# AndrewGYork/rescan_line_sted

Hardware: AMD Instinct MI355X
Metric: simulated frames/s (512x512, 20 RL iters) (higher is better)
Workload: dtype f32; 1 GPU; astronaut 128->512x512 (np.kron x4), point-descan STED PSF 107x107 (2.0x operating point), simulate (H + Philox Poisson) + 20 RL iterations per frame; n_psf=1, rl_iters=20, fft=576x576

## Files before the change

include/rlsted.h:

```cpp
#ifndef RLSTED_H
#define RLSTED_H

#include <stddef.h>
#include <stdint.h>

#ifdef __cplusplus
extern "C" {
#endif

#define RL_OK 0
#define RL_ERR_INVALID -1
#define RL_ERR_HIP -2
#define RL_ERR_UNSUPPORTED -3
#define RL_ERR_STATE -4

#define RL_F32 0
#define RL_F64 1

#define RL_RNG_NONE 0
#define RL_RNG_PHILOX 1

typedef struct rl_ctx rl_ctx;
typedef struct rl_deconv rl_deconv;
typedef struct rl_comm rl_comm;
// ... 44 lines not shown

int rl_deconv_get_object(rl_deconv* h, double* out);
int rl_deconv_get_noiseless(rl_deconv* h, double* out);
int rl_deconv_get_measurement(rl_deconv* h, double* out);
int rl_deconv_get_estimate(rl_deconv* h, double* out);
int rl_deconv_get_normalization(rl_deconv* h, double* out);

int rl_forward(rl_deconv* h, const double* x, double* out);
int rl_adjoint(rl_deconv* h, const double* y, double* out, int normalize);

int rl_deconv_last_ms(const rl_deconv* h, double* iterate_ms, double* simulate_ms);

int rl_deconv_bench_cycles(rl_deconv* h, int k, int reps, int rng_kind, uint64_t seed, double* total_ms);

int rl_deconv_device_ptr(rl_deconv* h, int which, void** ptr, size_t* n_elements, int* dtype);

int rl_deconv_measurement_written(rl_deconv* h);

int rl_deconv_strategy(const rl_deconv* h, int* separable, int* real_psf_spectrum, int* split_column_pass, int* frame_pairs);

int rl_deconv_object_classes(const rl_deconv* h, int* classes, int* shared_slices, int* slices);

int rl_deconv_simulated_images(const rl_deconv* h, int* images);

int rl_deconv_unresolved(rl_deconv* h, unsigned long long* count, int reset);

int rl_deconv_dims(const rl_deconv* h, int* batch, int* n_psf, int* ny, int* nx);

typedef struct rl_task {
    const double* object;
    double total_brightness;
    uint64_t seed;
    uint32_t image_id;
} rl_task;
int rl_batch_run(rl_deconv* h, const rl_task* tasks, int n_tasks, int k_iters, int rng_kind, double* estimates_out);

int rl_batch_submit(rl_deconv* h, const rl_task* tasks, int n_tasks, int k_iters, int rng_kind, void* dev_out, int out_dtype);

#define RL_TRACE_FIELDS 6
int rl_batch_submit_checkpoints(rl_deconv* h, const rl_task* tasks, int n_tasks, const int* k_list, int n_k, int rng_kind,
                                void* const* dev_out, int out_dtype, double* const* trace_dev);

int rl_device_alloc(rl_ctx* ctx, size_t bytes, void** dev_out);
int rl_device_free(rl_ctx* ctx, void* dev);
int rl_device_download(rl_ctx* ctx, const void* dev, int dtype, size_t n_elements, double* host_out);
int rl_device_upload(rl_ctx* ctx, void* dev, int dtype, size_t n_elements, const double* host);
// ... 121 lines not shown
```

rescan_line_sted_amd/_lib.py:

```python
import ctypes
import os

import numpy as np

_HERE = os.path.dirname(os.path.abspath(__file__))
LIB_PATH = os.environ.get('RLSTED_LIB') or os.path.join(_HERE, '_lib', 'librlsted.so')
DEFAULT_DEVICE = int(os.environ.get('RLSTED_DEVICE', '0'))

RL_F32, RL_F64 = 0, 1
RNG_NONE, RNG_PHILOX = 0, 1
DTYPES = {'f32': RL_F32, 'float32': RL_F32, 'f64': RL_F64, 'float64': RL_F64}
RL_ACCEL_NONE, RL_ACCEL_BIGGS_ANDREWS = 0, 1
ACCELERATIONS = {None: RL_ACCEL_NONE, 'none': RL_ACCEL_NONE, 'biggs-andrews': RL_ACCEL_BIGGS_ANDREWS}
RL_STOP_DISCREPANCY, RL_STOP_RELATIVE = 1, 2
STOP_RULES = {'discrepancy': RL_STOP_DISCREPANCY, 'relative': RL_STOP_RELATIVE}


def accel_mode(acceleration):
    try:
        return ACCELERATIONS[acceleration]
    except (KeyError, TypeError):
        raise ValueError("acceleration must be None or 'biggs-andrews'; got %r" % (acceleration,)) from None


# ... 32 lines not shown
    'rl_deconv_set_acceleration': (_i, [_vp, _i]),
    'rl_deconv_get_alpha': (_i, [_vp, _dp]),
    'rl_deconv_set_tv': (_i, [_vp, _c.c_double, _c.c_double]),
    'rl_deconv_get_tv': (_i, [_vp, _dp, _dp]),
    'rl_deconv_divergence': (_i, [_vp, _dp]),
    'rl_deconv_iterate_until': (_i, [_vp, _i, _i, _i, _c.c_double, _c.POINTER(_i), _dp, _c.POINTER(_i)]),
    'rl_deconv_get_object': (_i, [_vp, _dp]),
    'rl_deconv_get_noiseless': (_i, [_vp, _dp]),
    'rl_deconv_get_measurement': (_i, [_vp, _dp]),
    'rl_deconv_get_estimate': (_i, [_vp, _dp]),
    'rl_deconv_get_normalization': (_i, [_vp, _dp]),
    'rl_forward': (_i, [_vp, _dp, _dp]),
    'rl_adjoint': (_i, [_vp, _dp, _dp, _i]),
    'rl_deconv_last_ms': (_i, [_vp, _dp, _dp]),
    'rl_deconv_bench_cycles': (_i, [_vp, _i, _i, _i, _c.c_uint64, _dp]),
    'rl_deconv_time_kernels': (_i, [_vp, _i, _dp]),
    'rl_deconv_time_cycle': (_i, [_vp, _i, _i, _c.c_uint64, _dp, _dp, _dp]),
    'rl_deconv_device_ptr': (_i, [_vp, _i, _c.POINTER(_vp), _c.POINTER(_c.c_size_t), _c.POINTER(_i)]),
    'rl_host_alloc': (_i, [_c.c_size_t, _c.POINTER(_vp)]),
    'rl_host_free': (_i, [_vp]),
    'rl_deconv_strategy': (_i, [_vp, _c.POINTER(_i), _c.POINTER(_i), _c.POINTER(_i), _c.POINTER(_i)]),
    'rl_deconv_object_classes': (_i, [_vp, _c.POINTER(_i), _c.POINTER(_i), _c.POINTER(_i)]),
    'rl_deconv_simulated_images': (_i, [_vp, _c.POINTER(_i)]),
    'rl_deconv_unresolved': (_i, [_vp, _c.POINTER(_c.c_uint64), _i]),
    'rl_deconv_dims': (_i, [_vp, _c.POINTER(_i), _c.POINTER(_i), _c.POINTER(_i), _c.POINTER(_i)]),
    'rl_batch_run': (_i, [_vp, _vp, _i, _i, _i, _dp]),
    'rl_batch_submit': (_i, [_vp, _vp, _i, _i, _i, _vp, _i]),
    'rl_batch_submit_checkpoints': (_i, [_vp, _vp, _i, _c.POINTER(_i), _i, _i, _c.POINTER(_vp), _i, _c.POINTER(_vp)]),
    'rl_device_alloc': (_i, [_vp, _c.c_size_t, _c.POINTER(_vp)]),
    'rl_device_free': (_i, [_vp, _vp]),
    'rl_device_download': (_i, [_vp, _vp, _i, _c.c_size_t, _dp]),
    'rl_device_upload': (_i, [_vp, _vp, _i, _c.c_size_t, _dp]),
    'rl_comm_gather_device': (_i, [_vp, _vp, _c.POINTER(_c.c_size_t), _i, _i, _vp]),
    'rl_comm_bcast_host': (_i, [_vp, _dp, _c.c_size_t, _i]),
    'rl_comm_unique_id': (_i, [_vp]),
    'rl_comm_create': (_i, [_vp, _i, _i, _vp, _c.POINTER(_vp)]),
    'rl_comm_destroy': (_i, [_vp]),
    'rl_comm_info': (_i, [_vp, _c.POINTER(_i), _c.POINTER(_i)]),
    'rl_comm_barrier': (_i, [_vp]),
    'rl_comm_allreduce_max': (_i, [_vp, _dp]),
    'rl_gather': (_i, [_vp, _vp, _i, _i, _c.POINTER(_i), _dp]),
    'rl_gather_device': (_i, [_vp, _vp, _i, _i, _c.POINTER(_i), _c.POINTER(_vp), _c.POINTER(_c.c_size_t), _c.POINTER(_i)]),
    'rl_comm_gather_host': (_i, [_vp, _dp, _c.POINTER(_c.c_size_t), _i, _dp]),
    'rl_rotate_image': (_i, [_vp, _dp, _dp, _i, _i, _c.c_double, _i]),
    'rl_fig3_scan': (_i, [_vp, _vp, _dp, _dp, _c.POINTER(_i), _i, _c.POINTER(_i), _i, _dp, _dp, _dp, _dp]),
    'rl_gauss_fit': (_i, [_dp, _i, _dp, _c.POINTER(_i)]),
# ... 153 lines not shown

    def info(self):
        ly, lx, pitch, nbytes = _i(), _i(), _i(), _c.c_size_t()
        check(lib.rl_deconv_info(self.handle, ctypes.byref(ly), ctypes.byref(lx), ctypes.byref(pitch),
                                 ctypes.byref(nbytes)))
        return {'ly': ly.value, 'lx': lx.value, 'pitch': pitch.value, 'device_bytes': nbytes.value}

    def strategy(self):
        a, b, c, d = _i(), _i(), _i(), _i()
        check(lib.rl_deconv_strategy(self.handle, ctypes.byref(a), ctypes.byref(b), ctypes.byref(c), ctypes.byref(d)))
        return {'separable': a.value == 1, 'direct_stencil': a.value == 2, 'real_psf_spectrum': bool(b.value),
                'split_column_pass': bool(c.value), 'frame_pairs': bool(d.value)}

    def object_classes(self):
        a, b, c = _i(), _i(), _i()
        check(lib.rl_deconv_object_classes(self.handle, ctypes.byref(a), ctypes.byref(b), ctypes.byref(c)))
        return {'classes': a.value, 'shared_slices': b.value, 'slices': c.value}

    def simulated_images(self):
        a = _i()
        check(lib.rl_deconv_simulated_images(self.handle, ctypes.byref(a)))
        return a.value

    def set_object(self, obj, total_brightness=None):
        obj = as_f64(obj).reshape(self.B, self.ny, self.nx)
        tb = None
        if total_brightness is not None:
            tb = as_f64(np.broadcast_to(np.asarray(total_brightness, dtype=np.float64), (self.B,)))
        check(lib.rl_deconv_set_object(self.handle, ptr(obj), ptr(tb) if tb is not None else None))

    def simulate(self, seed=0, rng=RNG_PHILOX):
        check(lib.rl_deconv_simulate(self.handle, rng, _c.c_uint64(seed)))

    def unresolved(self, reset=False):
        n = _c.c_uint64(0)
        check(lib.rl_deconv_unresolved(self.handle, _c.byref(n), 1 if reset else 0))
        return int(n.value)

    def set_measurement(self, noisy):
        noisy = as_f64(noisy).reshape(self.B, self.V, self.ny, self.nx)
        check(lib.rl_deconv_set_measurement(self.handle, ptr(noisy)))

    def measurement_written(self):
        check(lib.rl_deconv_measurement_written(self.handle))

    def iterate(self, k=1):
# ... 175 lines not shown
```

rescan_line_sted_amd/csrc/aux_kernels.hip:

```cpp
#include <hip/hip_runtime.h>
#include "aux_kernels.hpp"
#include "philox_poisson.hpp"

namespace rl {

template <typename T>
__global__ void k_fill(T* p, size_t n, T value) {
    for (size_t i = (size_t)blockIdx.x * blockDim.x + threadIdx.x; i < n; i += (size_t)gridDim.x * blockDim.x) p[i] = value;
}

__global__ void k_psf_dft_rows(const double* __restrict__ psf, const double2* __restrict__ wx, double2* __restrict__ s1,
                               int py, int px, int lx, int kx) {
    const int k = blockIdx.x * blockDim.x + threadIdx.x;
    const int a = blockIdx.y, v = blockIdx.z;
    if (k >= kx) return;
    const int cx = (px - 1) / 2;
    const double* row = psf + ((size_t)v * py + a) * px;
    double re = 0.0, im = 0.0;
    for (int b = 0; b < px; ++b) {
        const int off = ((b - cx) % lx + lx) % lx;
        const double2 w = wx[(int)(((long long)k * off) % lx)];
        re += row[b] * w.x;
        im += row[b] * w.y;
    }
// ... 20 lines not shown
    if (transposed) {
        if (k < kx) out[((size_t)v * kx + k) * ly + ky] = mk<T>((T)(re * scale), (T)(im * scale));
    } else {
        out[((size_t)v * ly + ky) * pitch + k] = mk<T>((T)(re * scale), (T)(im * scale));
    }
}

struct PoissonKeys {
    unsigned long long seed0;
    unsigned image0, V;
    const unsigned long long* frame_seeds;
    const unsigned* frame_ids;
    const unsigned* rate_frame;
    __device__ __forceinline__ unsigned long long seed(unsigned img) const { return frame_seeds ? frame_seeds[img / V] : seed0; }
    __device__ __forceinline__ unsigned image(unsigned img) const {
        return frame_seeds ? frame_ids[img / V] * V + img % V : image0 + img;
    }
    template <typename T>
    __device__ __forceinline__ T rate(const T* __restrict__ noiseless, unsigned i, unsigned n_pix) const {
        if (!rate_frame) return noiseless[i];
        const unsigned img = i / n_pix, pix = i - img * n_pix;
        return noiseless[((size_t)rate_frame[img / V] * V + img % V) * n_pix + pix];
    }
};

constexpr int kPoissonE = 8, kPoissonTile = 256 * kPoissonE;
template <typename T>
__global__ void __launch_bounds__(256) k_poisson(const T* __restrict__ noiseless, T* __restrict__ noisy, unsigned n_pix, unsigned total,
                                                 PoissonKeys keys, int rng_kind) {
    __shared__ unsigned lst_idx[2][kPoissonTile];
    __shared__ T lst_lam[2][kPoissonTile];
    __shared__ unsigned cnt[2], cnt_small;
    const unsigned tid = threadIdx.x;
    for (unsigned tile0 = blockIdx.x * (unsigned)kPoissonTile; tile0 < total; tile0 += gridDim.x * (unsigned)kPoissonTile) {
        if (tid == 0) cnt[0] = cnt_small = 0;
        __syncthreads();
#pragma unroll
        for (int e = 0; e < kPoissonE; ++e) {
            const unsigned i = tile0 + tid + 256u * (unsigned)e;
            if (i < total) {
                const T lam_t = keys.rate(noiseless, i, n_pix);
                const double lam = (double)lam_t;
                if (rng_kind != 1) {
                    noisy[i] = (T)(lam + 1e-9);
                } else {
                    const unsigned img = i / n_pix, pix = i - img * n_pix;
                    double k;
                    if (philox_poisson_fast(lam, keys.seed(img), keys.image(img), pix, &k)) {
                        noisy[i] = (T)(k + 1e-9);
                    } else if (lam >= 10.0) {
                        const unsigned q = atomicAdd(&cnt[0], 1u);
                        lst_idx[0][q] = i;
                        lst_lam[0][q] = lam_t;
                    } else {
                        const unsigned q = kPoissonTile - 1u - atomicAdd(&cnt_small, 1u);
                        lst_idx[0][q] = i;
                        lst_lam[0][q] = lam_t;
                    }
                }
            }
        }
        __syncthreads();
        if (rng_kind != 1) continue;
        unsigned n = cnt[0];
        const unsigned n_small = cnt_small;
        int cur = 0;
        for (unsigned blk = 0; n > 0; ++blk) {
            if (tid == 0) cnt[cur ^ 1] = 0;
            __syncthreads();
            const bool last = blk + 1 == kPoissonMaxBlocks;
            for (unsigned q = tid; q < n; q += 256u) {
                const unsigned i = lst_idx[cur][q];
                const T lam_t = lst_lam[cur][q];
                const unsigned img = i / n_pix, pix = i - img * n_pix;
                const unsigned long long seed = keys.seed(img);
                double k;
                const bool done = philox_ptrs_attempt((double)lam_t, (unsigned)seed, (unsigned)(seed >> 32), keys.image(img), pix, blk, &k);
                if (done || last) {
                    noisy[i] = (T)((done || k >= 0.0 ? k : 0.0) + 1e-9);
                } else {
                    const unsigned q2 = atomicAdd(&cnt[cur ^ 1], 1u);
                    lst_idx[cur ^ 1][q2] = i;
                    lst_lam[cur ^ 1][q2] = lam_t;
                }
            }
            __syncthreads();
            n = cnt[cur ^ 1];
            cur ^= 1;
        }
        for (unsigned q = tid; q < n_small; q += 256u) {
            const unsigned at = kPoissonTile - 1u - q, i = lst_idx[0][at];
            const unsigned img = i / n_pix;
            noisy[i] = (T)(philox_poisson((double)lst_lam[0][at], keys.seed(img), keys.image(img), i - img * n_pix) + 1e-9);
        }
        __syncthreads();
    }
}

template <typename T>
__global__ void __launch_bounds__(1024) k_frame_sums(const T* __restrict__ x, size_t n, double* __restrict__ out) {
    __shared__ double part[16];
    const size_t chunks = gridDim.y, len = (n + chunks - 1) / chunks, i0 = blockIdx.y * len, i1 = i0 + len < n ? i0 + len : n;
    const T* f = x + (size_t)blockIdx.x * n;
    double v = 0.0;
    for (size_t i = i0 + threadIdx.x; i < i1; i += blockDim.x) v += (double)f[i];
    for (int off = 32; off > 0; off >>= 1) v += __shfl_down(v, off, 64);
    if ((threadIdx.x & 63) == 0) part[threadIdx.x >> 6] = v;
    __syncthreads();
    if (threadIdx.x < 64) {
        v = threadIdx.x < (blockDim.x >> 6) ? part[threadIdx.x] : 0.0;
        for (int off = 8; off > 0; off >>= 1) v += __shfl_down(v, off, 64);
        if (threadIdx.x == 0) out[(size_t)blockIdx.x * chunks + blockIdx.y] = v;
    }
}
template <typename T>
// ... 71 lines not shown
    if (e != hipSuccess) return e;
    const unsigned g = blocks_for(n, 256);
    if (dtype == DT_F32) k_split_real<float><<<g, 256, 0, s>>>((const cx<float>*)z, n, (float*)re, stats);
    else k_split_real<double><<<g, 256, 0, s>>>((const cx<double>*)z, n, (double*)re, stats);
    return hipGetLastError();
}

template <typename T>
__global__ void k_box_norm(const double* __restrict__ integ, T* __restrict__ out, int V, int py, int px, int ny, int nx) {
    const int j = blockIdx.x * blockDim.x + threadIdx.x, i = blockIdx.y;
    if (j >= nx) return;
    out[(size_t)i * nx + j] = box_norm_pixel<T>(integ, V, py, px, ny, nx, i, j);
}

hipError_t aux_box_norm(int dtype, const double* integral_dev, void* out, int V, int py, int px, int ny, int nx, hipStream_t s) {
    const dim3 grid((unsigned)((nx + 255) / 256), (unsigned)ny);
    if (dtype == DT_F32) k_box_norm<float><<<grid, 256, 0, s>>>(integral_dev, (float*)out, V, py, px, ny, nx);
    else k_box_norm<double><<<grid, 256, 0, s>>>(integral_dev, (double*)out, V, py, px, ny, nx);
    return hipGetLastError();
}

hipError_t aux_poisson(int dtype, const void* noiseless, void* noisy, unsigned n_pix, unsigned n_img, unsigned image0,
                       unsigned long long seed, int rng_kind, void* list_ws, hipStream_t s,
                       const unsigned long long* frame_seeds, const unsigned* frame_ids, unsigned V, const unsigned* rate_frame) {
    (void)list_ws;
    const PoissonKeys keys{seed, image0, V ? V : 1u, frame_seeds, frame_ids, rate_frame};
    const size_t total = (size_t)n_pix * n_img;
    if (total >= 0xffffffffull - (size_t)kPoissonTile * 4096) return hipErrorInvalidValue;
    if (total == 0) return hipSuccess;
    const size_t tiles = (total + kPoissonTile - 1) / kPoissonTile;
    const unsigned g = (unsigned)(tiles > 4096 ? 4096 : tiles);
    if (dtype == DT_F32) k_poisson<float><<<g, 256, 0, s>>>((const float*)noiseless, (float*)noisy, n_pix, (unsigned)total, keys, rng_kind);
    else k_poisson<double><<<g, 256, 0, s>>>((const double*)noiseless, (double*)noisy, n_pix, (unsigned)total, keys, rng_kind);
    return hipGetLastError();
}

hipError_t aux_scale_convert(int dtype, const double* src, void* dst, size_t n, size_t frames, const double* target,
                             double* sums, hipStream_t s, bool want_sums) {
    if (target || want_sums) frame_sums<double>(src, n, frames, sums, s);
    const unsigned g = blocks_for(n * frames, 256);
    if (dtype == DT_F32) k_scale_convert<float><<<g, 256, 0, s>>>(src, (float*)dst, n, frames, target, sums);
    else k_scale_convert<double><<<g, 256, 0, s>>>(src, (double*)dst, n, frames, target, sums);
    return hipGetLastError();
}

template <typename T>
__global__ void k_any_negative(const T* __restrict__ x, size_t n, int* __restrict__ flag) {
    bool neg = false;
    for (size_t i = (size_t)blockIdx.x * blockDim.x + threadIdx.x; i < n; i += (size_t)gridDim.x * blockDim.x) neg = neg || x[i] < (T)0;
    if (__any(neg) && (threadIdx.x & 63) == 0) atomicOr(flag, 1);
}
hipError_t aux_any_negative(int dtype, const void* src, size_t n, int* flag, hipStream_t s) {
    hipError_t e = hipMemsetAsync(flag, 0, sizeof(int), s);
    if (e != hipSuccess || n == 0) return e;
    const unsigned g = blocks_for(n, 256);
    if (dtype == DT_F32) k_any_negative<float><<<g, 256, 0, s>>>((const float*)src, n, flag);
// ... 74 lines not shown
```

rescan_line_sted_amd/csrc/aux_kernels.hpp:

```cpp
#pragma once
#include "fft_core.hpp"

#include <cstddef>

#if defined(__HIPCC__) || defined(__HIP_PLATFORM_AMD__)
#include <hip/hip_runtime.h>
#include "kernel_table.hpp"
#endif

namespace rl {

template <typename T>
RL_HD T box_norm_pixel(const double* __restrict__ integ, int V, int py, int px, int ny, int nx, int i, int j) {
    const int cy = (py - 1) / 2, cx = (px - 1) / 2;
    const int a0 = i + cy - ny + 1 > 0 ? i + cy - ny + 1 : 0, a1 = (i + cy < py - 1 ? i + cy : py - 1) + 1;
    const int b0 = j + cx - nx + 1 > 0 ? j + cx - nx + 1 : 0, b1 = (j + cx < px - 1 ? j + cx : px - 1) + 1;
    double acc = 0.0;
    if (a1 > a0 && b1 > b0) {
        for (int v = 0; v < V; ++v) {
            const double* I = integ + (size_t)v * (py + 1) * (px + 1);
            const double s = (I[(size_t)a1 * (px + 1) + b1] - I[(size_t)a0 * (px + 1) + b1]) - (I[(size_t)a1 * (px + 1) + b0] - I[(size_t)a0 * (px + 1) + b0]);
            acc += s > 0.0 ? s : 0.0;
        }
    }
    return (T)acc;
}

#if defined(__HIPCC__) || defined(__HIP_PLATFORM_AMD__)
hipError_t aux_fill(int dtype, void* p, size_t n, double value, hipStream_t s);
hipError_t aux_psf_spectrum(int dtype, const double* psf_dev, const void* wx_dev, const void* wy_dev, void* s1_dev,
                            void* out, int n_psf, int py, int px, int ly, int lx, int kx, int pitch, int transposed,
                            hipStream_t s);
size_t aux_poisson_workspace_bytes(size_t total_pixels);
hipError_t aux_poisson(int dtype, const void* noiseless, void* noisy, unsigned n_pix, unsigned n_img, unsigned image0,
                       unsigned long long seed, int rng_kind, void* list_ws, hipStream_t s,
                       const unsigned long long* frame_seeds = nullptr, const unsigned* frame_ids = nullptr, unsigned V = 1,
                       const unsigned* rate_frame = nullptr);
constexpr size_t kSumChunks = 64;
inline size_t aux_sums_elems(size_t frames) { return frames * (1 + kSumChunks); }
hipError_t aux_scale_convert(int dtype, const double* src, void* dst, size_t n, size_t frames, const double* target,
                             double* sums, hipStream_t s, bool want_sums = false);
hipError_t aux_any_negative(int dtype, const void* src, size_t n, int* flag, hipStream_t s);
hipError_t aux_image_sums(int dtype, const void* src, size_t n, size_t frames, double* sums, hipStream_t s);
hipError_t aux_scale_convert_indexed(int dtype, const double* src, const unsigned* idx, size_t n_unique, void* dst, size_t n, size_t frames,
                                     const double* target, double* sums, hipStream_t s);
hipError_t aux_to_f64(int dtype, const void* src, double* dst, size_t total, hipStream_t s);
hipError_t aux_cast(int dtype_src, const void* src, int dtype_dst, void* dst, size_t total, hipStream_t s);
hipError_t aux_gather_images(int dtype, const void* src, void* dst, const unsigned* list, size_t n, size_t images, unsigned V, hipStream_t s);
hipError_t aux_split_real(int dtype, const void* z, size_t n, void* re, double* stats, hipStream_t s);
hipError_t aux_box_norm(int dtype, const double* integral_dev, void* out, int V, int py, int px, int ny, int nx, hipStream_t s);
#endif
}
```

rescan_line_sted_amd/csrc/rlsted.cpp:

```cpp
#include "../../include/rlsted.h"

#include <hip/hip_runtime.h>

#include <cmath>
#include <cstdio>
#include <cstdlib>
#include <algorithm>
#include <cstring>
#include <map>
#include <string>
#include <vector>

#include "accel_kernels.hpp"
#include "aux_kernels.hpp"
#include "checkpoint_kernels.hpp"
#include "conv_kernels.hpp"
#include "kernel_table.hpp"
#include "object_classes.hpp"
#include "ctx.hpp"
#include "sep_kernels.hpp"
#include "sep_taps.hpp"
#include "stop_kernels.hpp"
#include "tv_kernels.hpp"

// ... 22 lines not shown

const KernelTable* table_for(int L) {
    switch (L) {
        case 64: return table_64();
        case 192: return table_192();
        case 256: return table_256();
        case 576: return table_576();
        case 1152: return table_1152();
        case 2304: return table_2304();
        case 4608: return table_4608();
    }
    return nullptr;
}
const int kLengths[] = {64, 192, 256, 576, 1152, 2304, 4608};

size_t esize(int dtype) { return dtype == RL_F32 ? 4 : 8; }

constexpr int kMaxLanes = 4;

struct PlanOptions {
    bool chunk_mb_set = false;
    double chunk_mb = 0;
    int lanes = 2;
    bool inplace = true;
    int col_order = 4;
    bool pair = false;
    double pair_max_ratio = 4.0;
    bool sub_one = false;
    int fuse_views = -1;
    bool col_split = true;
    bool real_psf = true;
    bool ones_shortcut = true;
    bool share_objects = true;
    int sep = 1;
    int sep_one = 1;
    int direct = 1;
    bool q_exp_est_set = false, q_exp_ratio_set = false;
    int q_exp_est = 14, q_exp_ratio = 14;
};

PlanOptions plan_options(int dtype, int n_psf) {
    PlanOptions o;
    auto flag = [](const char* name, bool unset) {
        const char* s = getenv(name);
        return s ? atoi(s) != 0 : unset;
    };
    auto number = [](const char* name, int unset, bool* set = nullptr) {
        const char* s = getenv(name);
        if (set) *set = s != nullptr;
        return s ? atoi(s) : unset;
    };
    if (const char* s = getenv("RLSTED_CHUNK_MB")) {
        o.chunk_mb_set = true;
        o.chunk_mb = atof(s);
    }
    o.lanes = std::min(std::max(number("RLSTED_LANES", o.lanes), 1), kMaxLanes);
    o.inplace = flag("RLSTED_INPLACE", o.inplace);
    o.col_order = std::max(number("RLSTED_COL_ORDER", o.col_order), 1);
    o.pair = flag("RLSTED_PAIR", dtype == RL_F32 && n_psf == 1);
    if (const char* s = getenv("RLSTED_PAIR_MAX_RATIO")) o.pair_max_ratio = atof(s);
    o.sub_one = flag("RLSTED_SUB_ONE", dtype == RL_F32 && RL_SPEC_QUANT == 0);
    if (const char* s = getenv("RLSTED_FUSE_VIEWS")) o.fuse_views = atoi(s) != 0 ? 1 : 0;
    o.col_split = flag("RLSTED_COL_SPLIT", o.col_split);
    o.real_psf = flag("RLSTED_REAL_PSF", o.real_psf);
    o.ones_shortcut = flag("RLSTED_ONES_SHORTCUT", o.ones_shortcut);
    o.share_objects = flag("RLSTED_SHARE_OBJECTS", o.share_objects);
    o.sep = number("RLSTED_SEP", o.sep);
    o.sep_one = number("RLSTED_SEP_ONE", o.sep_one);
    o.direct = number("RLSTED_DIRECT", o.direct);
    o.q_exp_est = number("RLSTED_Q_EXP_EST", o.q_exp_est, &o.q_exp_est_set);
    o.q_exp_ratio = number("RLSTED_Q_EXP_RATIO", o.q_exp_ratio, &o.q_exp_ratio_set);
    return o;
}

struct TempBuffers {
    std::vector<void*> bufs;
    int get(void** p, size_t bytes) {
        HIP_TRY(hipMalloc(p, bytes));
        bufs.push_back(*p);
// ... 588 lines not shown
        if (c > 8) {
            const int up = (c + 7) / 8 * 8;
            c = up <= fit ? up : std::max(8, fit / 8 * 8);
        }
        if (pair && (c & 1)) ++c;
        return c >= B ? B : c;
    }
    int start_estimate_chunk(int f0, int nf, bool with_spectrum = true) {
        HIP_TRY(aux_fill(dtype, off(est, (size_t)f0 * n_img()), (size_t)nf * n_img(), 1.0, cur()));
        if (with_spectrum && pair)
            RL_TRY(row_pair(ROW_FWD, nf, nullptr, pair_spec(f0), off(est, (size_t)f0 * n_img()), nullptr, nullptr));
        else if (with_spectrum && !sep)
            RL_TRY(row(ROW_FWD, (unsigned)nf, nullptr, off(spec_a, (size_t)f0 * n_spec() * 2), off(est, (size_t)f0 * n_img()),
                       nullptr, nullptr));
        return RL_OK;
    }
    int ensure_lanes() {
        if (fork) return RL_OK;
        HIP_TRY(hipEventCreateWithFlags(&fork, hipEventDisableTiming));
        for (int l = 0; l < opt.lanes; ++l) {
            HIP_TRY(hipStreamCreateWithFlags(&lane_stream[l], hipStreamNonBlocking));
            HIP_TRY(hipEventCreateWithFlags(&lane_done[l], hipEventDisableTiming));
            HIP_TRY(hipEventCreateWithFlags(&lane_drawn[l], hipEventDisableTiming));
        }
        HIP_TRY(hipEventCreateWithFlags(&rates_ready, hipEventDisableTiming));
        return RL_OK;
    }
    bool one_buffer() const { return V == 1 && opt.inplace; }
    void* est_spec(int f0) const { return pair ? pair_spec(f0) : off(spec_a, (size_t)f0 * n_spec() * 2); }
    void* ratio_spec(int f0) const { return pair || one_buffer() ? est_spec(f0) : off(spec_b, (size_t)f0 * V * n_spec() * 2); }
    void* parked(int f0) const { return off(spec_x, (size_t)f0 * V * n_spec_x() * 2); }
    bool ht_fused() const { return fuse_views && V > 1 && (col_split() || wave_private_y()); }
    int pass_h(const Iter& it) {
        if (it.first) return RL_OK;
        if (pair) return col_pair(est_spec(it.f0), ratio_spec(it.f0), (it.nf + 1) / 2, COL_H, &it);
        if (col_split() && split_h()) return col_split_pass(est_spec(it.f0), ratio_spec(it.f0), parked(it.f0), it.nf, COL_H, &it);
        return col(est_spec(it.f0), ratio_spec(it.f0), it.nf, COL_H, &it);
    }
    int pass_ratio(const Iter& it) {
        void* r = ratio_spec(it.f0);
        const void* m = off(meas, (size_t)it.f0 * V * n_img());
        if (pair) return row_pair(ROW_RATIO, it.nf, it.first ? spec_ones_pair : r, r, m, nullptr, nullptr, it.first ? 1 : 0, 1, &it);
        return row(ROW_RATIO, (unsigned)(it.nf * V), it.first ? spec_ones : r, r, m, nullptr, nullptr, nullptr, -1, it.first ? V : 0, &it);
    }
    int pass_ht(const Iter& it) {
        void* r = ratio_spec(it.f0);
// ... 30 lines not shown
        if (col_split()) RL_TRY(col_split_pass(sa, sb, parked(f0), nf, COL_H));
        else RL_TRY(col(sa, sb, nf, COL_H));
        RL_TRY(row(ROW_INV, (unsigned)(nf * V), sb, nullptr, nullptr, out, nullptr));
        return RL_OK;
    }
    std::vector<int> obj_class;
    int n_classes = 0;
    std::vector<SliceShare> share_slices;
    int share_cf = 0;
    std::vector<uint32_t> share_reps, share_rate;
    struct ShareLists { const unsigned *rep_frames, *rate_of; };
    ShareLists share_lists{nullptr, nullptr};
    unsigned* share_dev = nullptr;
    void *obj_c = nullptr, *noiseless_c = nullptr;
    void *cls_spec_a = nullptr, *cls_spec_b = nullptr, *cls_spec_x = nullptr;
    size_t share_cap = 0;
    int share_classes = 0;
    hipEvent_t rates_ready = nullptr;
    hipEvent_t lane_drawn[kMaxLanes] = {nullptr, nullptr, nullptr, nullptr};
    bool lane_drawn_set[kMaxLanes] = {false, false, false, false};
    int last_sim_images = 0;
    bool noiseless_sparse = false;
    int last_shared_slices = 0, last_slices = 0;
    bool share_possible() const { return opt.share_objects && !sep && (int)obj_class.size() == B && n_classes < B; }
    int build_share(int cf, const ShareLists* staged) {
        share_cf = 0;
        noiseless_sparse = false;
        share_classes = 0;
        share_layout(obj_class, cf, share_slices, share_reps, share_rate);
        const size_t total = (size_t)class_layout(obj_class, cf, share_slices, share_reps, share_rate);
        if (total > share_cap) {
            HIP_TRY(hipDeviceSynchronize());
            share_cap = 0;
            RL_TRY(release(&obj_c));
            RL_TRY(release(&noiseless_c));
            RL_TRY(release(&cls_spec_a));
            RL_TRY(release(&cls_spec_b));
            RL_TRY(release(&cls_spec_x));
            const size_t cap = (total + 7) / 8 * 8, sp = n_spec() * 2 * esize(dtype);
            RL_TRY(alloc(&obj_c, cap * n_img() * esize(dtype), SLACK));
            RL_TRY(alloc(&noiseless_c, cap * V * n_img() * esize(dtype), SLACK));
            if (!pair_layout) RL_TRY(alloc(&cls_spec_a, cap * sp, SLACK));
            RL_TRY(alloc(&cls_spec_b, cap * V * sp, SLACK));
            if (col_split()) {
                const size_t parked_bytes = cap * V * n_spec_x() * 2 * esize(dtype);
                RL_TRY(alloc(&cls_spec_x, parked_bytes));
// ... 66 lines not shown
        const int frames = std::min(f0 + nf, cp.nt) - f0;
        void* dst = cp.out ? cp.out[j] : nullptr;
        double* tr = cp.trace ? cp.trace[j] : nullptr;
        if (frames <= 0 || (!dst && !tr)) return RL_OK;
        const size_t o = (size_t)f0 * n_img();
        double* part = tr ? cp_part + (size_t)f0 * checkpoint_blocks(n_img(), esize(dtype)) * kCheckpointFields : nullptr;
        HIP_TRY(checkpoint_take(dtype, off(est, o), off(obj, o), cp.out_dtype, dst ? (char*)dst + o * esize(cp.out_dtype) : nullptr, part,
                                n_img(), frames, cur()));
        if (tr) HIP_TRY(checkpoint_totals(dtype, part, n_img(), frames, tr + (size_t)f0 * kCheckpointFields, cur()));
        return RL_OK;
    }
    int run_slices(int k, bool restart, const Draw* draw = nullptr, bool cycle_follows = false, const Checkpoints* cp = nullptr) {
        const int cf = chunk_frames();
        const int slices = (B + cf - 1) / cf;
        const int nl = slices < opt.lanes ? slices : opt.lanes;
        const bool keep_open = cycle_follows && nl > 1;
        if (accel && restart) RL_TRY(accel_reset());
        if (draw && share_possible() && share_cf != cf && !lanes_open) RL_TRY(build_share(cf, nullptr));
        const bool share = draw && share_possible() && share_cf == cf;
        if (nl > 1 && !lanes_open) {
            RL_TRY(ensure_lanes());
            HIP_TRY(hipEventRecord(fork, ctx->stream));
            for (int l = 0; l < nl; ++l) HIP_TRY(hipStreamWaitEvent(lane_stream[l], fork, 0));
        }
        if (draw) {
            const size_t stride = (aux_poisson_workspace_bytes((size_t)cf * V * n_img()) + 255) / 256 * 256;
            if (slice_ws_bytes < stride * slices) {
                HIP_TRY(hipDeviceSynchronize());
                slice_ws_bytes = 0;
                RL_TRY(release(&slice_ws));
                RL_TRY(alloc(&slice_ws, stride * slices));
                slice_ws_bytes = stride * slices;
            }
            slice_ws_stride = stride;
        }
        int rc = RL_OK;
        struct ActiveGuard {
            hipStream_t& a;
            ~ActiveGuard() { a = nullptr; }
        } active_guard{active};
        int shared_slices = 0, sim_images = 0;
        auto hip_rc = [&](hipError_t e, const char* what) -> int {
            return e == hipSuccess ? RL_OK : fail(RL_ERR_HIP, std::string(what) + ": " + hipGetErrorString(e));
        };
        bool lane_waits[kMaxLanes] = {false, false, false, false};
        int lane_last_shared[kMaxLanes] = {-1, -1, -1, -1};
        if (share && share_classes > 0) {
            active = nl > 1 ? lane_stream[0] : nullptr;
            for (int l = 0; l < kMaxLanes && rc == RL_OK; ++l) {
                if (!lane_drawn_set[l]) continue;
                lane_drawn_set[l] = false;
                rc = hip_rc(hipStreamWaitEvent(cur(), lane_drawn[l], 0), "class simulation");
            }
            if (rc == RL_OK) rc = forward_classes(share_classes);
            sim_images += share_classes * V;
            if (nl > 1 && rc == RL_OK) {
                rc = hip_rc(hipEventRecord(rates_ready, cur()), "class simulation");
                for (int l = 1; l < nl; ++l) lane_waits[l] = true;
                for (int sl = 0; sl < slices; ++sl)
                    if (share_slices[(size_t)sl].nrep > 0) lane_last_shared[sl % nl] = sl;
            }
        }
        auto simulate_slice = [&](int sl, int f0, int nf) -> int {
            const SliceShare ss = share ? share_slices[(size_t)sl] : SliceShare{};
            const void* rates = off(noiseless, (size_t)f0 * V * n_img());
            const int lane = nl > 1 ? sl % nl : 0;
            if (ss.nrep > 0) {
                if (lane_waits[lane]) {
                    HIP_TRY(hipStreamWaitEvent(cur(), rates_ready, 0));
                    lane_waits[lane] = false;
                }
                rates = noiseless_c;
                ++shared_slices;
            } else {
                RL_TRY(forward_slice(f0, nf));
                sim_images += nf * V;
            }
            void* ws = (char*)slice_ws + (size_t)sl * slice_ws_stride;
            TimedScope t(this, TK_POISSON, false);
            hipError_t e = aux_poisson(dtype, rates, off(meas, (size_t)f0 * V * n_img()),
                                       (unsigned)n_img(), (unsigned)(nf * V), (unsigned)(f0 * V), draw->seed, draw->rng_kind, ws, cur(),
                                       draw->key_seeds ? draw->key_seeds + f0 : nullptr, draw->key_ids ? draw->key_ids + f0 : nullptr, (unsigned)V,
                                       ss.nrep > 0 ? share_lists.rate_of + f0 : nullptr);
            if (e != hipSuccess) return fail(RL_ERR_HIP, std::string("Poisson kernels: ") + hipGetErrorString(e));
            if (lane_last_shared[lane] == sl) {
                HIP_TRY(hipEventRecord(lane_drawn[lane], cur()));
                lane_drawn_set[lane] = true;
            }
            return RL_OK;
        };
        for (int sl = 0, f0 = 0; f0 < B && rc == RL_OK; f0 += cf, ++sl) {
            const int nf = f0 + cf <= B ? cf : B - f0;
            active = nl > 1 ? lane_stream[sl % nl] : nullptr;
            if (draw) rc = simulate_slice(sl, f0, nf);
            const bool shortcut = restart && opt.ones_shortcut && spec_ones && k > 0 && !sep;
            const bool ones_first = shortcut && !accel && !tv_on();
            if (restart && rc == RL_OK && !ones_first) rc = start_estimate_chunk(f0, nf, !shortcut);
            const bool drop = pair && k >= 4;
            int cp_next = 0;
            for (int i = 0; i < k && rc == RL_OK; ++i) {
                if (accel) rc = accel_step(f0, nf, acc_steps + i, shortcut && i == 0, restart && i == 0);
                else if (tv_on()) rc = tv_iterate({f0, nf, shortcut && i == 0, restart && i == 0,  pair}, i > 0 || tv_sum_valid, true);
                else rc = iterate_chunk({f0, nf, shortcut && i == 0, restart && i == 0, drop && i == k - 1, ones_first && i == 0});
                if (cp && rc == RL_OK && cp_next < cp->n_k && cp->k_list[cp_next] == i + 1) rc = take_checkpoint(*cp, cp_next++, f0, nf);
            }
        }
        active = nullptr;
        if (nl > 1 && (!keep_open || rc != RL_OK)) {
            for (int l = 0; l < nl; ++l) {
                HIP_TRY(hipEventRecord(lane_done[l], lane_stream[l]));
                HIP_TRY(hipStreamWaitEvent(ctx->stream, lane_done[l], 0));
            }
            lanes_open = false;
        } else if (nl > 1) {
            lanes_open = true;
        }
        RL_TRY(rc);
        if (draw) {
            noiseless_sparse = shared_slices > 0;
            last_shared_slices = shared_slices;
            last_slices = slices;
            last_sim_images = sim_images;
        }
        if (restart) {
            est_ready = true;
            spec_valid = true;
            iterations = 0;
        }
        if (pair && k >= 4) spec_valid = false;
        if (accel) {
            spec_valid = false;
            acc_steps += k;
        }
        if (tv_on()) spec_valid = false;
        if (k > 0 || restart) tv_sum_valid = tv_on() && !accel && k > 0;
        iterations += k;
        return RL_OK;
    }
};

namespace rl {
// ... 74 lines not shown

int rl_deconv_destroy(rl_deconv* h) {
    if (!h) return RL_OK;
    (void)hipSetDevice(h->ctx->device);
    (void)hipStreamSynchronize(h->ctx->stream);
    for (hipStream_t s : h->lane_stream)
        if (s) (void)hipStreamSynchronize(s);
    if (h->copy_stream) (void)hipStreamSynchronize(h->copy_stream);
    for (const rl_deconv::Owned& o : h->owned) (void)hipFree(o.p);
    for (rl_deconv::BatchSlot& sl : h->bslot) {
        if (sl.host) (void)hipHostFree(sl.host);
        if (sl.uploaded) (void)hipEventDestroy(sl.uploaded);
        if (sl.freed) (void)hipEventDestroy(sl.freed);
    }
    if (h->copy_stream) (void)hipStreamDestroy(h->copy_stream);
    for (hipEvent_t e : h->event_pool) (void)hipEventDestroy(e);
    if (h->ev0) (void)hipEventDestroy(h->ev0);
    if (h->ev1) (void)hipEventDestroy(h->ev1);
    if (h->fork) (void)hipEventDestroy(h->fork);
    if (h->rates_ready) (void)hipEventDestroy(h->rates_ready);
    for (int l = 0; l < kMaxLanes; ++l) {
        if (h->lane_done[l]) (void)hipEventDestroy(h->lane_done[l]);
        if (h->lane_drawn[l]) (void)hipEventDestroy(h->lane_drawn[l]);
        if (h->lane_stream[l]) (void)hipStreamDestroy(h->lane_stream[l]);
    }
    delete h;
    return RL_OK;
}

static int build_psf_hat(rl_deconv* h, const double* psfs, void* hat, int width, int pitch, int transposed, void** re, double* imag_ratio) {
    rl_ctx* ctx = h->ctx;
    const size_t V = (size_t)h->V, np = V * h->py * h->px;
    {
        TempBuffers tmp;
        void *wy = nullptr, *wx = nullptr, *psf_dev = nullptr, *s1 = nullptr;
        RL_TRY(ctx->plain_twiddles(h->ly, &wy));
        RL_TRY(ctx->plain_twiddles(h->lx, &wx));
        RL_TRY(tmp.get(&psf_dev, np * 8));
        RL_TRY(tmp.get(&s1, V * h->py * width * 16));
        HIP_TRY(hipMemcpyAsync(psf_dev, psfs, np * 8, hipMemcpyHostToDevice, ctx->stream));
        HIP_TRY(aux_psf_spectrum(h->dtype, (const double*)psf_dev, wx, wy, s1, hat, h->V, h->py, h->px, h->ly, h->lx, width, pitch,
                                 transposed, ctx->stream));
        HIP_TRY(hipStreamSynchronize(ctx->stream));
    }
    if (!re) return RL_OK;
    TempBuffers tmp;
// ... 509 lines not shown
    HIP_TRY(hipEventRecord(h->ev1, s));
    HIP_TRY(hipEventSynchronize(h->ev1));
    float ms = 0;
    HIP_TRY(hipEventElapsedTime(&ms, h->ev0, h->ev1));
    *total_ms = ms;
    return RL_OK;
}


int rl_deconv_strategy(const rl_deconv* h, int* separable, int* real_psf_spectrum, int* split_column_pass, int* frame_pairs) {
    if (!h) return fail(RL_ERR_INVALID, "handle is NULL");
    if (frame_pairs) *frame_pairs = h->pair ? 1 : 0;
    if (separable) *separable = h->sep ? (h->sep_direct ? 2 : 1) : 0;
    if (real_psf_spectrum) *real_psf_spectrum = h->psf_hat_re ? 1 : 0;
    if (split_column_pass) *split_column_pass = !h->sep && !h->pair && h->col_split() ? 1 : 0;
    return RL_OK;
}

int rl_deconv_object_classes(const rl_deconv* h, int* classes, int* shared_slices, int* slices) {
    if (!h) return fail(RL_ERR_INVALID, "handle is NULL");
    if (classes) *classes = (int)h->obj_class.size() == h->B ? h->n_classes : 0;
    if (shared_slices) *shared_slices = h->last_shared_slices;
    if (slices) *slices = h->last_slices;
    return RL_OK;
}

int rl_deconv_simulated_images(const rl_deconv* h, int* images) {
    if (!h || !images) return fail(RL_ERR_INVALID, "NULL argument");
    *images = h->last_sim_images;
    return RL_OK;
}

int rl_deconv_unresolved(rl_deconv* h, unsigned long long* count, int reset) {
    if (!h || !count) return fail(RL_ERR_INVALID, "NULL argument");
    HIP_TRY(hipSetDevice(h->ctx->device));
    HIP_TRY(hipMemcpyAsync(count, h->unresolved, sizeof(unsigned long long), hipMemcpyDeviceToHost, h->ctx->stream));
    if (reset) HIP_TRY(hipMemsetAsync(h->unresolved, 0, sizeof(unsigned long long), h->ctx->stream));
    HIP_TRY(hipStreamSynchronize(h->ctx->stream));
    return RL_OK;
}

int rl_deconv_dims(const rl_deconv* h, int* batch, int* n_psf, int* ny, int* nx) {
    if (!h) return fail(RL_ERR_INVALID, "handle is NULL");
    if (batch) *batch = h->B;
    if (n_psf) *n_psf = h->V;
    if (ny) *ny = h->ny;
// ... 330 lines not shown
```

Before: 21550 frames/s.

## Add opt-in draw-ahead Poisson stream and per-tile image indexing in Poisson kernel

```diff
diff --git a/include/rlsted.h b/include/rlsted.h
--- a/include/rlsted.h
+++ b/include/rlsted.h
@@ -90,6 +90,8 @@
 int rl_deconv_object_classes(const rl_deconv* h, int* classes, int* shared_slices, int* slices);
 
 int rl_deconv_simulated_images(const rl_deconv* h, int* images);
+
+int rl_deconv_draws_ahead(const rl_deconv* h, int* slices);
 
 int rl_deconv_unresolved(rl_deconv* h, unsigned long long* count, int reset);
 
diff --git a/rescan_line_sted_amd/_lib.py b/rescan_line_sted_amd/_lib.py
--- a/rescan_line_sted_amd/_lib.py
+++ b/rescan_line_sted_amd/_lib.py
@@ -78,6 +78,7 @@
     'rl_deconv_strategy': (_i, [_vp, _c.POINTER(_i), _c.POINTER(_i), _c.POINTER(_i), _c.POINTER(_i)]),
     'rl_deconv_object_classes': (_i, [_vp, _c.POINTER(_i), _c.POINTER(_i), _c.POINTER(_i)]),
     'rl_deconv_simulated_images': (_i, [_vp, _c.POINTER(_i)]),
+    'rl_deconv_draws_ahead': (_i, [_vp, _c.POINTER(_i)]),
     'rl_deconv_unresolved': (_i, [_vp, _c.POINTER(_c.c_uint64), _i]),
     'rl_deconv_dims': (_i, [_vp, _c.POINTER(_i), _c.POINTER(_i), _c.POINTER(_i), _c.POINTER(_i)]),
     'rl_batch_run': (_i, [_vp, _vp, _i, _i, _i, _dp]),
@@ -277,6 +278,11 @@
         check(lib.rl_deconv_simulated_images(self.handle, ctypes.byref(a)))
         return a.value
 
+    def draws_ahead(self):
+        a = _i()
+        check(lib.rl_deconv_draws_ahead(self.handle, ctypes.byref(a)))
+        return a.value
+
     def set_object(self, obj, total_brightness=None):
         obj = as_f64(obj).reshape(self.B, self.ny, self.nx)
         tb = None
diff --git a/rescan_line_sted_amd/csrc/aux_kernels.hip b/rescan_line_sted_amd/csrc/aux_kernels.hip
--- a/rescan_line_sted_amd/csrc/aux_kernels.hip
+++ b/rescan_line_sted_amd/csrc/aux_kernels.hip
@@ -1,4 +1,5 @@
 #include <hip/hip_runtime.h>
+#include <type_traits>
 #include "aux_kernels.hpp"
 #include "philox_poisson.hpp"
 
@@ -66,29 +67,40 @@
         const unsigned img = i / n_pix, pix = i - img * n_pix;
         return noiseless[((size_t)rate_frame[img / V] * V + img % V) * n_pix + pix];
     }
+    template <typename T>
+    __device__ __forceinline__ const T* image_rates(const T* __restrict__ noiseless, unsigned img, unsigned n_pix) const {
+        return noiseless + (rate_frame ? (size_t)rate_frame[img / V] * V + img % V : (size_t)img) * n_pix;
+    }
 };
 
 constexpr int kPoissonE = 8, kPoissonTile = 256 * kPoissonE;
-template <typename T>
+template <typename T, bool TILE_IMG>
 __global__ void __launch_bounds__(256) k_poisson(const T* __restrict__ noiseless, T* __restrict__ noisy, unsigned n_pix, unsigned total,
                                                  PoissonKeys keys, int rng_kind) {
     __shared__ unsigned lst_idx[2][kPoissonTile];
     __shared__ T lst_lam[2][kPoissonTile];
     __shared__ unsigned cnt[2], cnt_small;
     const unsigned tid = threadIdx.x;
-    for (unsigned tile0 = blockIdx.x * (unsigned)kPoissonTile; tile0 < total; tile0 += gridDim.x * (unsigned)kPoissonTile) {
+    const unsigned n_tiles = (total + (unsigned)kPoissonTile - 1u) / (unsigned)kPoissonTile;
+    const unsigned turn = (unsigned)((float)gridDim.x * 0.6180339887f) | 1u;
+    for (unsigned first = 0, round = 0; first < n_tiles; first += gridDim.x, ++round) {
+        const unsigned tile = first + (blockIdx.x + round * turn) % gridDim.x;
+        if (tile >= n_tiles) continue;
+        const unsigned tile0 = tile * (unsigned)kPoissonTile;
         if (tid == 0) cnt[0] = cnt_small = 0;
         __syncthreads();
+        const unsigned img_t = TILE_IMG ? tile0 / n_pix : 0u;
+        const T* __restrict__ rates_t = TILE_IMG ? keys.image_rates(noiseless, img_t, n_pix) : nullptr;
 #pragma unroll
         for (int e = 0; e < kPoissonE; ++e) {
             const unsigned i = tile0 + tid + 256u * (unsigned)e;
             if (i < total) {
-                const T lam_t = keys.rate(noiseless, i, n_pix);
+                const T lam_t = TILE_IMG ? rates_t[i - img_t * n_pix] : keys.rate(noiseless, i, n_pix);
                 const double lam = (double)lam_t;
                 if (rng_kind != 1) {
                     noisy[i] = (T)(lam + 1e-9);
                 } else {
-                    const unsigned img = i / n_pix, pix = i - img * n_pix;
+                    const unsigned img = TILE_IMG ? img_t : i / n_pix, pix = i - img * n_pix;
                     double k;
                     if (philox_poisson_fast(lam, keys.seed(img), keys.image(img), pix, &k)) {
                         noisy[i] = (T)(k + 1e-9);
@@ -116,7 +128,7 @@
             for (unsigned q = tid; q < n; q += 256u) {
                 const unsigned i = lst_idx[cur][q];
                 const T lam_t = lst_lam[cur][q];
-                const unsigned img = i / n_pix, pix = i - img * n_pix;
+                const unsigned img = TILE_IMG ? img_t : i / n_pix, pix = i - img * n_pix;
                 const unsigned long long seed = keys.seed(img);
                 double k;
                 const bool done = philox_ptrs_attempt((double)lam_t, (unsigned)seed, (unsigned)(seed >> 32), keys.image(img), pix, blk, &k);
@@ -134,7 +146,7 @@
         }
         for (unsigned q = tid; q < n_small; q += 256u) {
             const unsigned at = kPoissonTile - 1u - q, i = lst_idx[0][at];
-            const unsigned img = i / n_pix;
+            const unsigned img = TILE_IMG ? img_t : i / n_pix;
             noisy[i] = (T)(philox_poisson((double)lst_lam[0][at], keys.seed(img), keys.image(img), i - img * n_pix) + 1e-9);
         }
         __syncthreads();
@@ -252,16 +264,23 @@
 
 hipError_t aux_poisson(int dtype, const void* noiseless, void* noisy, unsigned n_pix, unsigned n_img, unsigned image0,
                        unsigned long long seed, int rng_kind, void* list_ws, hipStream_t s,
-                       const unsigned long long* frame_seeds, const unsigned* frame_ids, unsigned V, const unsigned* rate_frame) {
+                       const unsigned long long* frame_seeds, const unsigned* frame_ids, unsigned V, const unsigned* rate_frame,
+                       unsigned grid_cap) {
     (void)list_ws;
     const PoissonKeys keys{seed, image0, V ? V : 1u, frame_seeds, frame_ids, rate_frame};
     const size_t total = (size_t)n_pix * n_img;
-    if (total >= 0xffffffffull - (size_t)kPoissonTile * 4096) return hipErrorInvalidValue;
+    if (total >= 0xffffffffull - (size_t)kPoissonTile * kPoissonGrid) return hipErrorInvalidValue;
     if (total == 0) return hipSuccess;
     const size_t tiles = (total + kPoissonTile - 1) / kPoissonTile;
-    const unsigned g = (unsigned)(tiles > 4096 ? 4096 : tiles);
-    if (dtype == DT_F32) k_poisson<float><<<g, 256, 0, s>>>((const float*)noiseless, (float*)noisy, n_pix, (unsigned)total, keys, rng_kind);
-    else k_poisson<double><<<g, 256, 0, s>>>((const double*)noiseless, (double*)noisy, n_pix, (unsigned)total, keys, rng_kind);
+    const size_t cap = grid_cap < 1 ? 1 : grid_cap > kPoissonGrid ? kPoissonGrid : grid_cap;
+    const unsigned g = (unsigned)(tiles > cap ? cap : tiles);
+    const bool tile_img = n_pix % (unsigned)kPoissonTile == 0;
+    auto launch = [&](auto zero, auto in_image) {
+        using T = decltype(zero);
+        k_poisson<T, decltype(in_image)::value><<<g, 256, 0, s>>>((const T*)noiseless, (T*)noisy, n_pix, (unsigned)total, keys, rng_kind);
+    };
+    if (dtype == DT_F32) tile_img ? launch(0.0f, std::true_type{}) : launch(0.0f, std::false_type{});
+    else tile_img ? launch(0.0, std::true_type{}) : launch(0.0, std::false_type{});
     return hipGetLastError();
 }
 
diff --git a/rescan_line_sted_amd/csrc/aux_kernels.hpp b/rescan_line_sted_amd/csrc/aux_kernels.hpp
--- a/rescan_line_sted_amd/csrc/aux_kernels.hpp
+++ b/rescan_line_sted_amd/csrc/aux_kernels.hpp
@@ -32,10 +32,11 @@
                             void* out, int n_psf, int py, int px, int ly, int lx, int kx, int pitch, int transposed,
                             hipStream_t s);
 size_t aux_poisson_workspace_bytes(size_t total_pixels);
+constexpr unsigned kPoissonGrid = 4096;
 hipError_t aux_poisson(int dtype, const void* noiseless, void* noisy, unsigned n_pix, unsigned n_img, unsigned image0,
                        unsigned long long seed, int rng_kind, void* list_ws, hipStream_t s,
                        const unsigned long long* frame_seeds = nullptr, const unsigned* frame_ids = nullptr, unsigned V = 1,
-                       const unsigned* rate_frame = nullptr);
+                       const unsigned* rate_frame = nullptr, unsigned grid_cap = kPoissonGrid);
 constexpr size_t kSumChunks = 64;
 inline size_t aux_sums_elems(size_t frames) { return frames * (1 + kSumChunks); }
 hipError_t aux_scale_convert(int dtype, const double* src, void* dst, size_t n, size_t frames, const double* target,
diff --git a/rescan_line_sted_amd/csrc/rlsted.cpp b/rescan_line_sted_amd/csrc/rlsted.cpp
--- a/rescan_line_sted_amd/csrc/rlsted.cpp
+++ b/rescan_line_sted_amd/csrc/rlsted.cpp
@@ -68,6 +68,8 @@
     bool chunk_mb_set = false;
     double chunk_mb = 0;
     int lanes = 2;
+    bool draw_ahead = false;
+    int draw_grid = 128;
     bool inplace = true;
     int col_order = 4;
     bool pair = false;
@@ -101,6 +103,8 @@
         o.chunk_mb = atof(s);
     }
     o.lanes = std::min(std::max(number("RLSTED_LANES", o.lanes), 1), kMaxLanes);
+    o.draw_ahead = flag("RLSTED_DRAW_AHEAD", o.draw_ahead);
+    o.draw_grid = std::min(std::max(number("RLSTED_DRAW_GRID", o.draw_grid), 1), (int)kPoissonGrid);
     o.inplace = flag("RLSTED_INPLACE", o.inplace);
     o.col_order = std::max(number("RLSTED_COL_ORDER", o.col_order), 1);
     o.pair = flag("RLSTED_PAIR", dtype == RL_F32 && n_psf == 1);
@@ -735,6 +739,8 @@
             HIP_TRY(hipStreamCreateWithFlags(&lane_stream[l], hipStreamNonBlocking));
             HIP_TRY(hipEventCreateWithFlags(&lane_done[l], hipEventDisableTiming));
             HIP_TRY(hipEventCreateWithFlags(&lane_drawn[l], hipEventDisableTiming));
+            HIP_TRY(hipEventCreateWithFlags(&lane_begun[l], hipEventDisableTiming));
+            HIP_TRY(hipEventCreateWithFlags(&drawn_ahead[l], hipEventDisableTiming));
         }
         HIP_TRY(hipEventCreateWithFlags(&rates_ready, hipEventDisableTiming));
         return RL_OK;
@@ -811,6 +817,10 @@
     int last_sim_images = 0;
     bool noiseless_sparse = false;
     int last_shared_slices = 0, last_slices = 0;
+    hipStream_t draw_stream() const { return ctx->stream; }
+    hipEvent_t lane_begun[kMaxLanes] = {nullptr, nullptr, nullptr, nullptr}, drawn_ahead[kMaxLanes] = {nullptr, nullptr, nullptr, nullptr};
+    bool lane_begun_set[kMaxLanes] = {false, false, false, false};
+    int last_draws_ahead = 0;
     bool share_possible() const { return opt.share_objects && !sep && (int)obj_class.size() == B && n_classes < B; }
     int build_share(int cf, const ShareLists* staged) {
         share_cf = 0;
@@ -923,7 +933,15 @@
             RL_TRY(ensure_lanes());
             HIP_TRY(hipEventRecord(fork, ctx->stream));
             for (int l = 0; l < nl; ++l) HIP_TRY(hipStreamWaitEvent(lane_stream[l], fork, 0));
-        }
+            for (bool& b : lane_begun_set) b = false;
+        }
+        const bool ahead = opt.draw_ahead && share && share_classes > 0 && nl > 1 && slices > nl;
+        std::vector<char> on_draw_stream((size_t)slices, 0);
+        for (int sl = 0; ahead && sl < slices; ++sl) {
+            const int on_lane = (slices - sl % nl + nl - 1) / nl;
+            on_draw_stream[(size_t)sl] = share_slices[(size_t)sl].nrep > 0 && (sl >= nl || (lane_begun_set[sl] && on_lane >= 2));
+        }
+        int draws_ahead = 0;
         if (draw) {
             const size_t stride = (aux_poisson_workspace_bytes((size_t)cf * V * n_img()) + 255) / 256 * 256;
             if (slice_ws_bytes < stride * slices) {
@@ -947,7 +965,7 @@
         bool lane_waits[kMaxLanes] = {false, false, false, false};
         int lane_last_shared[kMaxLanes] = {-1, -1, -1, -1};
         if (share && share_classes > 0) {
-            active = nl > 1 ? lane_stream[0] : nullptr;
+            active = ahead ? draw_stream() : nl > 1 ? lane_stream[0] : nullptr;
             for (int l = 0; l < kMaxLanes && rc == RL_OK; ++l) {
                 if (!lane_drawn_set[l]) continue;
                 lane_drawn_set[l] = false;
@@ -957,20 +975,39 @@
             sim_images += share_classes * V;
             if (nl > 1 && rc == RL_OK) {
                 rc = hip_rc(hipEventRecord(rates_ready, cur()), "class simulation");
-                for (int l = 1; l < nl; ++l) lane_waits[l] = true;
+                for (int l = ahead ? 0 : 1; l < nl; ++l) lane_waits[l] = true;
                 for (int sl = 0; sl < slices; ++sl)
-                    if (share_slices[(size_t)sl].nrep > 0) lane_last_shared[sl % nl] = sl;
+                    if (share_slices[(size_t)sl].nrep > 0 && !on_draw_stream[(size_t)sl]) lane_last_shared[sl % nl] = sl;
             }
         }
         auto simulate_slice = [&](int sl, int f0, int nf) -> int {
             const SliceShare ss = share ? share_slices[(size_t)sl] : SliceShare{};
             const void* rates = off(noiseless, (size_t)f0 * V * n_img());
             const int lane = nl > 1 ? sl % nl : 0;
+            if (on_draw_stream[(size_t)sl]) {
+                hipStream_t lane_s = cur();
+                active = draw_stream();
+                hipError_t e = hipStreamWaitEvent(draw_stream(), lane_begun[lane], 0);
+                if (e == hipSuccess) {
+                    TimedScope t(this, TK_POISSON, false);
+                    e = aux_poisson(dtype, noiseless_c, off(meas, (size_t)f0 * V * n_img()), (unsigned)n_img(), (unsigned)(nf * V),
+                                    (unsigned)(f0 * V), draw->seed, draw->rng_kind, nullptr, draw_stream(),
+                                    draw->key_seeds ? draw->key_seeds + f0 : nullptr, draw->key_ids ? draw->key_ids + f0 : nullptr,
+                                    (unsigned)V, share_lists.rate_of + f0, (unsigned)opt.draw_grid);
+                }
+                active = lane_s;
+                if (e != hipSuccess) return fail(RL_ERR_HIP, std::string("Poisson kernels: ") + hipGetErrorString(e));
+                HIP_TRY(hipEventRecord(drawn_ahead[lane], draw_stream()));
+                HIP_TRY(hipStreamWaitEvent(lane_s, drawn_ahead[lane], 0));
+                ++shared_slices;
+                ++draws_ahead;
+                return RL_OK;
+            }
+            if ((ss.nrep > 0 || ahead) && lane_waits[lane]) {
+                HIP_TRY(hipStreamWaitEvent(cur(), rates_ready, 0));
+                lane_waits[lane] = false;
+            }
             if (ss.nrep > 0) {
-                if (lane_waits[lane]) {
-                    HIP_TRY(hipStreamWaitEvent(cur(), rates_ready, 0));
-                    lane_waits[lane] = false;
-                }
                 rates = noiseless_c;
                 ++shared_slices;
             } else {
@@ -994,6 +1031,10 @@
             const int nf = f0 + cf <= B ? cf : B - f0;
             active = nl > 1 ? lane_stream[sl % nl] : nullptr;
             if (draw) rc = simulate_slice(sl, f0, nf);
+            if (ahead && rc == RL_OK) {
+                rc = hip_rc(hipEventRecord(lane_begun[sl % nl], cur()), "draw ahead");
+                lane_begun_set[sl % nl] = rc == RL_OK;
+            }
             const bool shortcut = restart && opt.ones_shortcut && spec_ones && k > 0 && !sep;
             const bool ones_first = shortcut && !accel && !tv_on();
             if (restart && rc == RL_OK && !ones_first) rc = start_estimate_chunk(f0, nf, !shortcut);
@@ -1018,6 +1059,7 @@
         }
         RL_TRY(rc);
         if (draw) {
+            last_draws_ahead = draws_ahead;
             noiseless_sparse = shared_slices > 0;
             last_shared_slices = shared_slices;
             last_slices = slices;
@@ -1138,6 +1180,8 @@
     for (int l = 0; l < kMaxLanes; ++l) {
         if (h->lane_done[l]) (void)hipEventDestroy(h->lane_done[l]);
         if (h->lane_drawn[l]) (void)hipEventDestroy(h->lane_drawn[l]);
+        if (h->lane_begun[l]) (void)hipEventDestroy(h->lane_begun[l]);
+        if (h->drawn_ahead[l]) (void)hipEventDestroy(h->drawn_ahead[l]);
         if (h->lane_stream[l]) (void)hipStreamDestroy(h->lane_stream[l]);
     }
     delete h;
@@ -1693,6 +1737,12 @@
     if (classes) *classes = (int)h->obj_class.size() == h->B ? h->n_classes : 0;
     if (shared_slices) *shared_slices = h->last_shared_slices;
     if (slices) *slices = h->last_slices;
+    return RL_OK;
+}
+
+int rl_deconv_draws_ahead(const rl_deconv* h, int* slices) {
+    if (!h || !slices) return fail(RL_ERR_INVALID, "NULL argument");
+    *slices = h->last_draws_ahead;
     return RL_OK;
 }
 
```

Result: faster. 21780 frames/s, median of 6 (+1.1%).
